# aouyang1/go-muse

Measured on AMD Instinct MI355X. Metric: series-pairs XCorr/sec at N=4096, 1M-series batch; achieved HBM GB/s, higher is better.
Workload: dtype f64

## Files before the change

### go-muse_amd/binding.py

```python
import ctypes
import os

import numpy as np

from . import build as _build

_i32 = ctypes.c_int32
_i64 = ctypes.c_int64
_f64 = ctypes.c_double
_vp = ctypes.c_void_p
_dp = ctypes.POINTER(ctypes.c_double)
_i32p = ctypes.POINTER(ctypes.c_int32)
_i64p = ctypes.POINTER(ctypes.c_int64)

MUSE_OK = 0
MUSE_ERR_INVALID = -1
MUSE_ERR_LENGTH = -2
MUSE_ERR_ZERO_STD = -3
MUSE_ERR_NO_DEVICE = -4
MUSE_ERR_HIP = -5
MUSE_ERR_UNSUPPORTED = -6
MUSE_ERR_NOMEM = -7
MUSE_ERR_EMPTY = -8
MUSE_LAG_WINDOW_MAX = 63
# ... 61 lines not shown
    "muse_merge_group_winners": (ctypes.c_int, [_recp, ctypes.POINTER(ctypes.c_uint8), _i32, _i32, _recp, ctypes.POINTER(ctypes.c_uint8)]),
    "muse_merge_records": (ctypes.c_int, [_recp, _i64, _i32, _i64p, _i32p, _dp, _i32p, _dp]),
    "muse_batch_score_many": (ctypes.c_int, [ctypes.POINTER(_vp), _i32]),
    "muse_batch_read_scores": (ctypes.c_int, [_vp, _i32p, _dp]),
    "muse_batch_last_run_info": (ctypes.c_int, [_vp, _i32p, _i64p]),
    "muse_batch_last_run_path": (ctypes.c_int, [_vp, _i32p]),
    "muse_batch_kernel_name": (ctypes.c_int, [_vp, ctypes.c_char_p, _i32]),
    "muse_test_set_screen_bound_scale": (ctypes.c_int, [_vp, _f64]),
    "muse_test_screen_bound": (ctypes.c_int, [_i32, _f64, _dp]),
    "muse_test_wave_argmax": (ctypes.c_int, [_vp, _dp, _dp, _dp]),
    "muse_test_rows_always_copy": (ctypes.c_int, [_vp, _i32]),
    "muse_test_pool_stats": (ctypes.c_int, [_vp, _i64p, _i64p, _i64p, _i64p]),
    "muse_test_xcorr_repeat": (ctypes.c_int, [_vp, _i32]),
    "muse_test_huge_batch_mb": (ctypes.c_int, [_vp, _i32]),
    "muse_test_clock_probe_start": (ctypes.c_int, [_vp, _f64, _f64]),
    "muse_test_clock_probe_stop": (ctypes.c_int, [_vp]),
    "muse_test_clock_probe_read": (ctypes.c_int, [_vp, _dp, _i32, _i32p]),
    "muse_batch_screen_estimates": (ctypes.c_int, [_vp, _i32, _dp, ctypes.POINTER(ctypes.c_uint32), _dp]),
    "muse_batch_score_many_windowed": (ctypes.c_int, [ctypes.POINTER(_vp), _i32, _i32]),
    "muse_batch_run_many_windowed": (ctypes.c_int, [ctypes.POINTER(_vp), _i32, _i32p, _i32, _i32, _i32, _f64, _i32, _i32,
                                                    _i64p, _i32p, _dp, _i32p, _dp]),
    "muse_test_window_many_plan": (ctypes.c_int, [_i32, _i32, _i32p, _i32p, _i32p, _i32p, _i32p, _i32p]),
    "muse_batch_run_many": (ctypes.c_int, [ctypes.POINTER(_vp), _i32, _i32p, _i32, _i32, _i32, _f64, _i32, _i32,
                                           _i64p, _i32p, _dp, _i32p, _dp]),
    "muse_batch_free": (ctypes.c_int, [_vp]),
    "muse_xcorr_with_x": (ctypes.c_int, [_vp, _dp, _dp, _i32, _i32, _dp, _i32p, _dp, _i32p]),
    "muse_xcorr": (ctypes.c_int, [_vp, _dp, _i32, _dp, _i32, _i32, _i32, _dp, _i32p, _dp, _i32p]),
    "muse_xcorr_groups": (ctypes.c_int, [_vp, _vp, _i32, _i32, _i32p, _dp, _i32p, _dp]),
    "muse_xcorr_batch": (ctypes.c_int, [_vp, _dp, _dp, _i64, _i32, _i32, _i32, _i32, _i32p, _dp, _i32p, _dp]),
    "muse_ctx_set_spectrum_cache": (ctypes.c_int, [_vp, _i32]),
    "muse_group_spectrum_cache": (ctypes.c_int, [_vp, _i64p, _i64p]),
    "muse_group_drop_spectrum_cache": (ctypes.c_int, [_vp]),
    "muse_test_spectrum_cache_limits": (ctypes.c_int, [_vp, _i64, _i64]),
    "muse_test_spectrum_cache_policy": (ctypes.c_int, [_i64, _i32, _i32, _i32, _i64, _i64, _i64, _i32p, _i64p, _i64p]),
    "muse_test_batch_redo_pairs": (ctypes.c_int, [_vp, _i64p, _i64, _i64p]),
    "muse_next_pow2": (_i64, [_f64]),
}


class MuseError(RuntimeError):
    def __init__(self, status, message):
        super().__init__("muse_hip status %d: %s" % (status, message))
        self.status = status
        self.message = message


_lib = None


def lib_path():
    return _build.LIB


def load():
    global _lib
    if _lib is None:
        path = lib_path()
        if not os.path.exists(path):
            raise MuseError(MUSE_ERR_NO_DEVICE,
                            "%s is not built; run `python -c 'import __graft_entry__ as g; g.build()'`" % path)
        L = ctypes.CDLL(path)
        for name, (res, args) in SIGNATURES.items():
            fn = getattr(L, name)
            fn.restype = res
            fn.argtypes = args
        _lib = L
# ... 28 lines not shown
```

### go-muse_amd/csrc/capi_batch.hip

```cpp
#include "capi_internal.h"
#include "xcorr_huge.h"

using namespace muse;


int ilog2(int64_t n)
{
    int l = 0;
    while (((int64_t)1 << l) < n)
        l++;
    return l;
}

int build_spectrum(muse_ctx *ctx, const double *ref_host, int N, int n, int normalize, double x_scale,
                          double xc_scale, double2 *X, double2 *xc, float2 *xcf, double *xs, int *zero_std)
{
    double *dref = nullptr;
    int *dstat = nullptr;
    double2 *dscr = nullptr;
    HIP_TRY(dmalloc(ctx, &dref, (size_t)N * sizeof(double)));
    hipError_t e = dmalloc(ctx, &dstat, sizeof(int));
    if (e == hipSuccess && n > GENERIC_LDS_MAX_N)
        e = dmalloc(ctx, &dscr, (size_t)n * sizeof(double2));
    if (e == hipSuccess)
// ... 467 lines not shown
        return fail(MUSE_ERR_INVALID, "NULL group");
    std::lock_guard<std::mutex> lock(g->ready_mu);
    if (rows_cached)
        *rows_cached = (g->zc_state == muse_group::ZC_VALID && g->zc_rewrites == g->rewrites) ? g->zc_rows : 0;
    if (bytes)
        *bytes = g->zc_bytes;
    return MUSE_OK;
}

extern "C" int muse_group_drop_spectrum_cache(muse_group *g)
{
    if (!g)
        return fail(MUSE_ERR_INVALID, "NULL group");
    std::lock_guard<std::mutex> lock(g->ready_mu);
    if (g->zc_segs.empty() && g->zc_state == muse_group::ZC_NONE)
        return MUSE_OK;
    int rc = use_device(g->ctx);
    if (rc)
        return rc;
    HIP_TRY(hipStreamSynchronize(g->ctx->stream));
    group_drop_spectrum_cache(g);
    return MUSE_OK;
}

extern "C" int muse_test_spectrum_cache_limits(muse_ctx *ctx, int64_t min_rows, int64_t budget_bytes)
{
    if (!ctx)
        return fail(MUSE_ERR_INVALID, "NULL context");
    ctx->zc_min_rows.store(min_rows < 0 ? ZC_MIN_ROWS : min_rows);
    ctx->zc_budget.store(budget_bytes < 0 ? -1 : budget_bytes);
    return MUSE_OK;
}

extern "C" int muse_test_spectrum_cache_policy(int64_t rows, int32_t N, int32_t f32, int32_t mode, int64_t min_rows,
                                               int64_t free_bytes, int64_t budget_bytes, int32_t *decision,
                                               int64_t *rows_cached, int64_t *bytes)
{
    if (!decision || !rows_cached || !bytes)
        return fail(MUSE_ERR_INVALID, "NULL output");
    *decision = spectrum_cache_policy(rows, N, f32 != 0, mode, min_rows < 0 ? ZC_MIN_ROWS : min_rows, free_bytes,
                                      budget_bytes < 0 ? -1 : budget_bytes, rows_cached, bytes);
    return MUSE_OK;
}

extern "C" int muse_test_batch_redo_pairs(muse_batch *b, int64_t *pairs, int64_t cap, int64_t *count)
{
    if (!b || !count || cap < 0 || (cap > 0 && !pairs))
        return fail(MUSE_ERR_INVALID, "bad redo-list arguments");
    *count = 0;
    int rc = use_device(b->ctx);
    if (rc)
        return rc;
    HIP_TRY(hipStreamSynchronize(b->stream()));
    if (!b->ovf_count || !b->ovf_list.p)
        return MUSE_OK;
    int listed = 0;
    HIP_TRY(hipMemcpy(&listed, b->ovf_count, sizeof(int), hipMemcpyDeviceToHost));
    *count = listed;
    const int64_t k = std::min<int64_t>(std::min<int64_t>(listed, cap), b->ovf_list.cap);
    if (k > 0)
        HIP_TRY(hipMemcpy(pairs, b->ovf_list.p, (size_t)k * sizeof(long long), hipMemcpyDeviceToHost));
    return MUSE_OK;
}

extern "C" int muse_batch_score(muse_batch *b)
{
// ... 42 lines not shown
        p.gsmall = kc.gsmall;
    if (variant == KERNEL_GENERIC && b->n <= GENERIC_LDS_MAX_N)
        p.gscratch = nullptr;
    LaunchTimer timer(ctx, false, st);
    LaunchTimer redo_timer(ctx, true, st);
    if (variant == KERNEL_R16_FOLD) {
        HIP_TRY(b->ovf_list.ensure(ctx, 2 * p.npairs, st));
        p.ovf_count = b->ovf_count;
        p.work_counter = b->ovf_count + 1;
        p.ovf_list = b->ovf_list.p;
        HIP_TRY(hipMemsetAsync(b->ovf_count, 0, 2 * sizeof(int), st));
        ZcPlan plan;
        std::unique_lock<std::mutex> zc_lock(b->g->ready_mu, std::defer_lock);
        if (allow_spectrum_cache && spectrum_cache_candidate(b, variant)) {
            zc_lock.lock();
            rc = plan_spectrum_cache(b, plan);
            if (rc)
                return rc;
            if (!plan.use)
                zc_lock.unlock();
        }
        HIP_TRY(timer.begin());
        if (plan.use) {
            bool launched = false;
            const auto next_launch = [&]() {
                const hipError_t e = launched ? hipMemsetAsync(b->ovf_count + 1, 0, sizeof(int), st) : hipSuccess;
                launched = true;
                return e;
            };
            for (const auto &sg : plan.readers) {
                FusedParams r = p;
                r.npairs = sg.pairs;
                HIP_TRY(next_launch());
                HIP_TRY(launch_cached(r, SpectrumCacheArgs{sg.zc(), sg.zstat(), sg.pair0, sg.pairs}, ctx->num_cus, st));
            }
            if (plan.tail_pair0 < p.npairs) {
                FusedParams w = p;
                w.npairs = p.npairs - plan.tail_pair0;
                HIP_TRY(next_launch());
                HIP_TRY(launch_cache_fill(w, SpectrumCacheArgs{plan.tail_zpairs ? plan.tail_seg.zc() : nullptr,
                                                               plan.tail_zpairs ? plan.tail_seg.zstat() : nullptr,
                                                               plan.tail_pair0, plan.tail_zpairs}, ctx->num_cus, st));
            }
            zc_lock.unlock();
        } else {
            HIP_TRY(launch_fused(p, variant, ctx->num_cus, st));
        }
        HIP_TRY(timer.end());
        FusedParams q = p;
        q.pair_list = b->ovf_list.p;
        q.pair_count = b->ovf_count;
        q.dense_total = ctx->variant == 0 ? p.npairs : 0;
        q.npairs = std::min<long long>(p.npairs, (long long)ctx->num_cus * 3);
        HIP_TRY(redo_timer.begin());
        HIP_TRY(launch_fused(q, KERNEL_R16_OCC3, ctx->num_cus, st));
        HIP_TRY(redo_timer.end());
        if (p.npairs >= 1024 && !(b->handoff_host && b->handoff_M == M && b->handoff_rewrites == b->g->rewrites)) {
            if (!b->handoff_host)
                HIP_TRY(hmalloc(ctx, &b->handoff_host, sizeof(int)));
            *b->handoff_host = 0;
            b->handoff_M = M;
            b->handoff_rewrites = b->g->rewrites;
            HIP_TRY(hipMemcpyAsync(b->handoff_host, b->ovf_count, sizeof(int), hipMemcpyDeviceToHost, st));
        }
    } else if (variant == KERNEL_LONG) {
        HIP_TRY(b->ovf_list.ensure(ctx, 2 * p.npairs, st));
        p.ovf_count = b->ovf_count;
// ... 28 lines not shown
    if (!lag || !mv)
        return fail(MUSE_ERR_INVALID, "NULL output");
    HIP_TRY(hipMemcpyAsync(lag, b->lag.p, (size_t)M * sizeof(int), hipMemcpyDeviceToHost, b->stream()));
    HIP_TRY(hipMemcpyAsync(mv, b->mv.p, (size_t)M * sizeof(double), hipMemcpyDeviceToHost, b->stream()));
    HIP_TRY(hipStreamSynchronize(b->stream()));
    return MUSE_OK;
}

extern "C" int muse_batch_kernel_name(muse_batch *b, char *name, int32_t cap)
{
    if (!b || !name || cap < 1)
        return fail(MUSE_ERR_INVALID, "NULL argument");
    char k[96] = "xcorr_fused_generic";
    const char *padded = b->N < b->n ? "true" : "false", *f32 = b->g->f32 ? "true" : "false";
    if (b->many_tiles > 0) {
        snprintf(k, sizeof(k), "xcorr_window_many_mfma<%d, %s>", b->many_tiles, window_wide(b->g->rows, b->g->stride) ? "true" : "false");
    } else if (b->windowed()) {
        const int L = std::min(b->lag_window, b->n / 2);
        snprintf(k, sizeof(k), "xcorr_window_mfma<%d, %s>", (2 * L + 1 + 15) / 16,
                 window_wide(b->g->rows, b->g->stride) ? "true" : "false");
    } else if (b->n > GENERIC_MAX_N) {
        snprintf(k, sizeof(k), "huge_rows<false>");
    } else {
        const KernelChoice kc = choose_kernel(b, (b->g->M + 1) / 2);
        switch (kc.error ? -1 : kc.variant) {
        case KERNEL_R16_FOLD: {
            bool cached = false;
            if (spectrum_cache_candidate(b, kc.variant)) {
                std::lock_guard<std::mutex> lock(b->g->ready_mu);
                int64_t rc_ = 0, by_ = 0;
                cached = b->g->zc_state == muse_group::ZC_VALID && b->g->zc_rewrites == b->g->rewrites && b->g->zc_rows > 0 &&
                         spectrum_cache_policy(b->g->M, b->N, false, b->ctx->zc_mode.load(), b->ctx->zc_min_rows.load(), 0, 0, &rc_, &by_) != ZC_POLICY_NONE;
            }
            if (cached)
                snprintf(k, sizeof(k), "xcorr_cached_n4096<%s>", padded);
            else
                snprintf(k, sizeof(k), "xcorr_fused_n4096_fold<false, %s, %s>", padded, f32);
            break;
        }
        case KERNEL_R16_OCC3: snprintf(k, sizeof(k), "xcorr_fused_n4096_occ4"); break;
        case KERNEL_SMALL: snprintf(k, sizeof(k), "xcorr_fused_small<%d, %s, false, %s>", b->logn, padded, f32); break;
        case KERNEL_LONG: snprintf(k, sizeof(k), "xcorr_fused_long<%d, %s, false>", b->logn, padded); break;
        case KERNEL_STOCKHAM: snprintf(k, sizeof(k), b->n >= 8192 ? "xcorr_fused_stk_4step" : "xcorr_fused_stockham"); break;
        case KERNEL_REAL_SPLIT: snprintf(k, sizeof(k), "xcorr_fused_real32k_split<%s>", padded); break;
        case KERNEL_REAL: snprintf(k, sizeof(k), "xcorr_fused_real%dk<%s>", b->n / 1024, padded); break;
        default: break;
        }
    }
    snprintf(name, (size_t)cap, "%s", k);
    return MUSE_OK;
}

extern "C" int muse_batch_free(muse_batch *b)
{
    if (!b)
        return MUSE_OK;
    muse_ctx *const c = b->ctx;
    (void)hipSetDevice(c->device);
    (void)hipStreamSynchronize(b->stream());
    if (b->sp && b->sp->refs.fetch_sub(1) == 1) {
        dfree(c, b->sp->X);
        dfree(c, b->sp->xc);
        dfree(c, b->sp->xcp);
        dfree(c, b->sp->xcw);
        dfree(c, b->sp->xcf);
        dfree(c, b->sp->xs);
        dfree(c, b->sp->c1);
        delete b->sp;
// ... 43 lines not shown
```

### go-muse_amd/csrc/capi_internal.h

```cpp
#pragma once
#include <hip/hip_runtime.h>

#include <algorithm>
#include <atomic>
#include <mutex>
#include <cmath>
#include <cstdarg>
#include <cstdio>
#include <cstdlib>
#include <cstring>
#include <ctime>
#include <limits>
#include <map>
#include <new>
#include <string>
#include <unordered_map>
#include <utility>
#include <vector>

#include "muse_hip.h"
#include "muse_hip_test.h"
#include "xcorr_kernels.h"

using namespace muse;
// ... 73 lines not shown
    std::vector<double *> stage_pool;
    std::mutex stage_mu;
    PoolBuf<double2> zscratch;
    PoolBuf<void *> many_tab;
    std::vector<void *> many_host;
    double screen_delta = 1e-4;
    int screening = 0;
    int64_t screen_min_rows = 0;
    double screen_e_scale = 1.0;
    int variant = 0;
    int xcorr_repeat = 1;
    unsigned long long *dbg_stamps = nullptr;
    hipStream_t probe_stream = nullptr;
    unsigned long long *probe_buf = nullptr;
    bool timing = false;
    std::vector<std::pair<hipEvent_t, hipEvent_t>> events, redo_events;
    double total_ms = 0.0, redo_ms = 0.0;
    int64_t launches = 0, redo_launches = 0;
    char pci[32] = {0};
    MemPool dev_pool, host_pool;
    HugeWork huge;
    int huge_batch_mb = 0;
    std::mutex huge_mu;
    std::mutex small_mu;
    std::vector<std::pair<unsigned char *, int>> small_free;
    unsigned long long small_token = 0;
    std::mutex timing_mu;
    std::atomic<bool> rows_always_copy{false};
    std::vector<void *> rows_slots;
    std::mutex rows_mu;
    std::atomic<int> zc_mode{1};
    std::atomic<int64_t> zc_min_rows{ZC_MIN_ROWS};
    std::atomic<int64_t> zc_budget{-1};
    std::atomic<int> win_rows_slices{0};
    std::atomic<bool> gather_nt{false};
    std::atomic<int> refs{1};
};

struct muse_group {
    std::atomic<int> refs{1};
    muse_ctx *ctx = nullptr;
    double *rows = nullptr;
    float *rows32 = nullptr;
    bool f32 = false;
    size_t elem() const { return f32 ? sizeof(float) : sizeof(double); }
    void *base() const { return f32 ? (void *)rows32 : (void *)rows; }
    int64_t cap = 0, M = 0, stride = 0;
    PoolBuf<double> hstats;
    int64_t hstats_rows = 0;
    uint64_t rewrites = 0;
    std::vector<void *> retired;
    int32_t N = 0;
    double *stage[2] = {nullptr, nullptr};
    hipEvent_t stage_done[2] = {nullptr, nullptr};
    int cur = 0;
    int64_t staged = 0;
    int64_t flushed = 0;
    int64_t stage_rows = 0;
    int small_appends = 0;
    int64_t win_rows = 0, win_committed = 0;
    std::mutex win_mu;
    hipEvent_t uploaded = nullptr;
    bool upload_pending = false;
    std::mutex ready_mu;
    HostBuf<long long> gidx_host;
    PoolBuf<long long> gidx_dev;
// ... 191 lines not shown
```

### go-muse_amd/csrc/foldk_device.h

```cpp
#pragma once
#include <hip/hip_runtime.h>
#include <stdint.h>

#include "fold_device.h"
#include "r16_device.h"

namespace muse {

namespace foldk {

using namespace occ4;
using namespace fold;

constexpr int XW = 544;

template <int PERM>
__device__ __forceinline__ constexpr int pr(int k)
{
    return PERM ? BR16(k) : k;
}

template <int MODE, int PERM, bool TAILBAR = false>
__device__ __forceinline__ void exchange_cross(double2 (&v)[16], double2 *xbuf, const int wave, const int t_, const int wcol = -1)
{
// ... 143 lines not shown
                 : [w0] "=&v"(w[0]), [w1] "=&v"(w[1]), [w2] "=&v"(w[2]), [w3] "=&v"(w[3]), [w4] "=&v"(w[4]),
                   [w5] "=&v"(w[5]), [w6] "=&v"(w[6]), [w7] "=&v"(w[7]), [w8] "=&v"(w[8]), [w9] "=&v"(w[9]),
                   [w10] "=&v"(w[10]), [w11] "=&v"(w[11]), [w12] "=&v"(w[12]), [w13] "=&v"(w[13]),
                   [w14] "=&v"(w[14]), [w15] "=&v"(w[15]), [sv] "=&s"(sv)
                 : [ra] "v"(raddr), [wa] "v"(waddr), [m] "s"(first), [d0] "v"(d[0]), [d1] "v"(d[1]), [d2] "v"(d[2]),
                   [d3] "v"(d[3]), [d4] "v"(d[4]), [d5] "v"(d[5]), [d6] "v"(d[6]), [d7] "v"(d[7])
                 : "memory", "scc");
#pragma unroll
    for (int e = 0; e < 16; e++)
        v[e] = make_double2(w[e].x, w[e].y);
}

struct G2Fetch {
    const double2 *p;
    int j;
    __device__ __forceinline__ double2 operator()(int s) const { return p[16 * s + j]; }
};
struct G3Fetch {
    const double2 *p;
    int t;
    __device__ __forceinline__ double2 operator()(int s) const
    {
        return ldg2(scalar_ptr_at(p, ((s + 1) & ~1) * 256), t - 256 * (s & 1));
    }
};

struct G3Derived {
    double2 g[8];
    __device__ __forceinline__ static double2 sq(const double2 w) { return make_double2(fma_(w.x, w.x, -(w.y * w.y)), (w.x + w.x) * w.y); }
    __device__ __forceinline__ static double2 mulc(const double2 w, const double c, const double s)
    {
        return make_double2(fma_(w.y, s, w.x * c), fma_(-w.x, s, w.y * c));
    }
    __device__ __forceinline__ G3Derived(const double2 *tab, int t)
    {
        constexpr double H = 0.70710678118654752440;
        const double2 w8 = G3Fetch{tab, t}(2), w16 = G3Fetch{tab, t}(4);
        g[2] = w8;
        g[4] = w16;
        g[1] = sq(w8);
        g[0] = sq(g[1]);
        g[3] = make_double2(H * (w8.x + w8.y), H * (w8.y - w8.x));
        g[5] = mulc(w16, C16_1, S16_1);
        g[6] = make_double2(H * (w16.x + w16.y), H * (w16.y - w16.x));
        g[7] = mulc(w16, S16_1, C16_1);
    }
    __device__ __forceinline__ double2 operator()(int s) const { return g[s]; }
};

template <typename F>
__device__ __forceinline__ void gdft16_nr_l2(double2 (&v)[16], F fetch)
{
    double2 ga[4], gb[4];
#pragma unroll
    for (int s = 0; s < 4; s++)
        ga[s] = fetch(s);
    gdft16_nr_s12(v, ga[0], ga[1]);
    fence();
#pragma unroll
    for (int s = 0; s < 4; s++)
        gb[s] = fetch(4 + s);
    fence();
    gdft16_nr_s3(v, ga[2], ga[3]);
    fence();
    fence();
    gdft16_nr_s4(v, gb[0], gb[1], gb[2], gb[3]);
}

constexpr int REC = 36;

// ... 192 lines not shown
```

### go-muse_amd/csrc/xcorr_kernels.h

```cpp
#pragma once
#include <hip/hip_runtime.h>
#include <stdint.h>

#include "muse_hip.h"

namespace muse {

enum { KERNEL_GENERIC = 0, KERNEL_R16_OCC3 = 6, KERNEL_STOCKHAM = 10, KERNEL_R16_FOLD = 11, KERNEL_SMALL = 12, KERNEL_LONG = 13, KERNEL_REAL = 14, KERNEL_REAL_SPLIT = 15 };

struct FusedParams {
    const double *rows;
    const float *rows32;
    long long M;
    long long stride;
    long long npairs;
    int N;
    int n;
    int logn;
    int normalize_y;
    const double2 *xc;
    const double2 *tw1;
    const double2 *tw2;
    const double2 *xcp;
    const double2 *g2;
// ... 38 lines not shown
    const long long *pair_list;
    const int *pair_count;
    long long dense_total;
    long long gscratch_slices;
    const double *xrows;
    long long xstride;
    int Nx;
    double invN, invNm1;
};
inline FusedParams with_reciprocals(FusedParams p)
{
    p.invN = 1.0 / (double)p.N;
    p.invNm1 = 1.0 / (double)(p.N - 1);
    return p;
}

hipError_t launch_fused(const FusedParams &p, int variant, int num_cus, hipStream_t stream);
hipError_t launch_fused_occ4(const FusedParams &p, int num_cus, hipStream_t stream);
hipError_t launch_screen_pass(const FusedParams &p, int num_cus, hipStream_t stream);
hipError_t launch_screen_pass_many(const FusedParams &p, int num_cus, hipStream_t stream);
hipError_t launch_screen_pass_stk(const FusedParams &p, int num_cus, hipStream_t stream);
enum : unsigned { SCR_IN = 1u, SCR_OUT = 2u, SCR_POS = 4u, SCR_NEG = 8u, SCR_REFINE = 16u, SCR_NAN = 32u };
hipError_t launch_fused_fold(const FusedParams &p, int num_cus, hipStream_t stream);
hipError_t launch_fused_multi(const FusedParams &p, int num_cus, hipStream_t stream);
constexpr int ZC_STAT = 16;
constexpr long long ZC_PAIR_BYTES = 4096 * 16 + ZC_STAT * 8;
struct SpectrumCacheArgs {
    double2 *zc;
    double *zstat;
    long long pair0;
    long long zpairs;
};
hipError_t launch_cache_fill(const FusedParams &p, const SpectrumCacheArgs &c, int num_cus, hipStream_t stream);
hipError_t launch_cached(const FusedParams &p, const SpectrumCacheArgs &c, int num_cus, hipStream_t stream);
hipError_t launch_fused_small(const FusedParams &p, int num_cus, hipStream_t stream);
hipError_t launch_fused_stockham(const FusedParams &p, int num_cus, hipStream_t stream);
hipError_t launch_fused_long(const FusedParams &p, int num_cus, hipStream_t stream);
hipError_t launch_real_split_tables(const double2 *xc, double2 *out, hipStream_t stream);
hipError_t launch_real8k_tables(const double2 *xc, double2 *out, hipStream_t stream);
hipError_t launch_two_sided_real(const FusedParams &p, int num_cus, hipStream_t stream);
hipError_t launch_fused_real_split(const FusedParams &p, int num_cus, hipStream_t stream);
hipError_t launch_fused_real(const FusedParams &p, int num_cus, hipStream_t stream);
hipError_t launch_two_sided(const FusedParams &p, int num_cus, hipStream_t stream);
hipError_t launch_two_sided_small(const FusedParams &p, int num_cus, hipStream_t stream);
hipError_t launch_lane_order_rows(const double2 *in, double2 *out, int R1, hipStream_t stream);
hipError_t launch_lane_order(const double2 *in, double2 *out, hipStream_t stream);
hipError_t launch_indicator_corr(const double *xs, int n, int pad, double *c1, hipStream_t stream);
hipError_t launch_ref_spectrum(const double *ref_dev, int N, int n, int logn, int normalize, double x_scale,
                               double xc_scale, const double2 *twm, double2 *X, double2 *xc, float2 *xcf, double *xs,
                               double2 *gscratch, int *status, hipStream_t stream);
constexpr int SMALL_MAX_N = 16384;
constexpr int GENERIC_LDS_MAX_N = 8192;
constexpr int GENERIC_MAX_N = 65536;
constexpr int GENERIC_GLOBAL_WGS_PER_CU = 2;
constexpr int STOCKHAM_GLOBAL_WGS_PER_CU = 2;
constexpr int LONG_WGS_PER_CU = 4;
constexpr int GSCRATCH_SLICES_PER_CU = 4;
static_assert(LONG_WGS_PER_CU <= GSCRATCH_SLICES_PER_CU && GENERIC_GLOBAL_WGS_PER_CU <= GSCRATCH_SLICES_PER_CU &&
                  2 * STOCKHAM_GLOBAL_WGS_PER_CU <= GSCRATCH_SLICES_PER_CU,
              "the scratch buffer is sized for GSCRATCH_SLICES_PER_CU slices per CU");
constexpr int WIN_KC = 1024;
constexpr int WIN_E_TAIL = 128;
static_assert(2 * MUSE_LAG_WINDOW_MAX + 2 <= WIN_E_TAIL, "the staged image covers every lag of the widest window");
struct WindowParams {
    const double *rows;
    long long M, stride;
    int N;
// ... 143 lines not shown
```

### go-muse_amd/csrc/xcorr_r16_cached.hip

```cpp
#include <hip/hip_runtime.h>
#include <stdint.h>
#include <algorithm>

#include "foldk_device.h"

namespace muse {

namespace foldk {

#if defined(__HIP_DEVICE_COMPILE__)
typedef d2v __attribute__((address_space(1))) *zc_out_ptr;
typedef double __attribute__((address_space(1))) *zstat_out_ptr;
typedef const double __attribute__((address_space(4))) *zstat_in_ptr;
#endif

__device__ __forceinline__ void finalize_prev(const double *prec, const int wave, const int lane, const double invN,
                                              const double invNm1, const FusedParams &p)
{
    if (lane == 0 && wave < 2 && prec[34] >= 0.0 && (wave == 0 || prec[35] != 0.0)) {
        const long long row = (long long)prec[34] + wave;
        if (finalize(prec, wave, invN, invNm1, p.mv + row, p.lag + row)) {
            const int slot = atomicAdd(p.ovf_count, 1);
            p.ovf_list[slot] = row >> 1;
        }
    }
}

}

template <bool PADDED>
__global__ __launch_bounds__(OCC_THREADS, 4) void xcorr_cache_fill_n4096(const FusedParams p, const SpectrumCacheArgs c)
{
    using namespace occ4;
    using namespace fold;
    using namespace foldk;
    __shared__ double2 xbuf[OCC_XBUF];
    __shared__ double2 g2s[128];
    __shared__ double red[2 * REC];
    __shared__ int next_s[2];
    const int t = threadIdx.x;
    const int lane = t & 63;
    const int wave = __builtin_amdgcn_readfirstlane(t >> 6);
    double2 *const xw = xbuf + XW * wave;
    const int pad = PADDED ? 4096 - p.N : 0;
    const double invN = PADDED ? p.invN : 1.0 / 4096.0, invNm1 = PADDED ? p.invNm1 : 1.0 / 4095.0;

// ... 108 lines not shown
                    cq[k] = c1l(8 * h + k);
                fence();
#pragma unroll
                for (int k = 0; k < 8; k++) {
                    const int r = BR16(8 * h + k);
                    v[r] = make_double2(fma(-mA, cq[k], v[r].x), fma(-mB, cq[k], v[r].y));
                }
            }
        }
        wave_argmax_store(v, wave, lane, rec + 6 * wave);
        fence();
        request_rows(nxt);
        fence();
        if (wave == 0 && lane == 0) {
            rec[32] = s1a;
            rec[33] = s1b;
        }
        parity ^= 1;
    }
    lds_barrier();
    {
        const double *const prec = red + REC * (parity ^ 1);
        if (t < 2 && prec[34] >= 0.0 && (t == 0 || prec[35] != 0.0)) {
            const long long row = (long long)prec[34] + t;
            if (finalize(prec, t, invN, invNm1, p.mv + row, p.lag + row)) {
                const int slot = atomicAdd(p.ovf_count, 1);
                p.ovf_list[slot] = row >> 1;
            }
        }
    }
}

template <bool PADDED>
__global__ __launch_bounds__(OCC_THREADS, 4) void xcorr_cached_n4096(const FusedParams p, const SpectrumCacheArgs c)
{
    using namespace occ4;
    using namespace fold;
    using namespace foldk;
    __shared__ double2 xbuf[OCC_XBUF];
    __shared__ double2 g2s[128];
    __shared__ double red[2 * REC];
    __shared__ int next_s[2];
    const int t = threadIdx.x;
    const int lane = t & 63;
    const int wave = __builtin_amdgcn_readfirstlane(t >> 6);
    double2 *const xw = xbuf + XW * wave;
    const double invN = PADDED ? p.invN : 1.0 / 4096.0, invNm1 = PADDED ? p.invNm1 : 1.0 / 4095.0;

    if (t < 128)
        g2s[t] = p.g2[t];
    if (t < 2)
        red[REC * (t) + 34] = -1.0;
    __syncthreads();
    const auto tl = [&]() __attribute__((always_inline)) {
        int x = t;
        if (PADDED)
            asm volatile("" : "+v"(x));
        return x;
    };

    int parity = 0;
    const long long first = c.pair0, total = c.pair0 + p.npairs;
    d2v zn[16];
    const auto request_z = [&](long long pr) __attribute__((always_inline)) {
#pragma unroll
        for (int i = 0; i < 16; i++)
            zn[i] = __builtin_nontemporal_load((gptr<d2v>)scalar_ptr_at(c.zc, (pr - first) * 4096 + 256 * ((i + 1) & ~1)) + (t - 256 * (i & 1)));
    };
    request_z(first + blockIdx.x < total ? first + (long long)blockIdx.x : first);

    long long nextpair = 0;
    for (long long pair = first + blockIdx.x; pair < total; pair = nextpair) {
        const long long rA = 2 * pair;
        const bool hasB = rA + 1 < p.M;
        double *const rec = red + REC * parity;
        const double *const prec = red + REC * (parity ^ 1);
        if (t == 0)
            next_s[parity] = (int)gridDim.x + atomicAdd(p.work_counter, 1);
        double st[10];
#if defined(__HIP_DEVICE_COMPILE__)
        {
            const zstat_in_ptr sp = (zstat_in_ptr)(unsigned long long)(c.zstat + (pair - first) * ZC_STAT);
#pragma unroll
            for (int k = 0; k < 10; k++)
                st[k] = sp[k];
        }
#endif
        double2 v[16];
#pragma unroll
        for (int i = 0; i < 16; i++)
            v[i] = make_double2(zn[i].x, zn[i].y);
        xc_stage1(v, [&](int j) __attribute__((always_inline)) {
            return ldg2(scalar_ptr_at(p.xcp, 256 * ((j + 1) & ~1)), t - 256 * (j & 1));
        });
        dft16_rn_s234(v);
        exchange_local<0>(v, xw, tl());
        gdft16_nr(v, G2Fetch{g2s, t & 15});
// ... 18 lines not shown
#pragma unroll
            for (int h = 0; h < 2; h++) {
                double cq[8];
#pragma unroll
                for (int k = 0; k < 8; k++)
                    cq[k] = c1l(8 * h + k);
                fence();
#pragma unroll
                for (int k = 0; k < 8; k++) {
                    const int r = BR16(8 * h + k);
                    v[r] = make_double2(fma(-mA, cq[k], v[r].x), fma(-mB, cq[k], v[r].y));
                }
            }
        }
        wave_argmax_store(v, wave, lane, rec + 6 * wave);
        fence();
        request_z(nxt);
        fence();
        parity ^= 1;
    }
    lds_barrier();
    {
        const double *const prec = red + REC * (parity ^ 1);
        if (t < 2 && prec[34] >= 0.0 && (t == 0 || prec[35] != 0.0)) {
            const long long row = (long long)prec[34] + t;
            if (finalize(prec, t, invN, invNm1, p.mv + row, p.lag + row)) {
                const int slot = atomicAdd(p.ovf_count, 1);
                p.ovf_list[slot] = row >> 1;
            }
        }
    }
}

static bool cache_launch_ok(const FusedParams &p, const SpectrumCacheArgs &c)
{
    return p.rows && !p.rows32 && p.n == 4096 && p.N > 2048 && p.N <= 4096 && p.npairs > 0 && c.pair0 >= 0 &&
           2 * (c.pair0 + p.npairs) <= p.M + 1 && p.work_counter && p.ovf_count && p.ovf_list && p.g2 && p.g3a && p.g3b && p.xcp &&
           (p.N == 4096 || p.c1);
}

hipError_t launch_cache_fill(const FusedParams &p_in, const SpectrumCacheArgs &c, int num_cus, hipStream_t stream)
{
    const FusedParams p = with_reciprocals(p_in);
    if (!cache_launch_ok(p, c) || c.zpairs < 0 || c.zpairs > p.npairs || (c.zpairs > 0 && (!c.zc || !c.zstat)) ||
        2 * (c.pair0 + c.zpairs) > p.M)
        return hipErrorInvalidValue;
    const dim3 g((unsigned)std::min<long long>(p.npairs, (long long)num_cus * 4)), b(OCC_THREADS);
    if (p.N < 4096)
        hipLaunchKernelGGL((xcorr_cache_fill_n4096<true>), g, b, 0, stream, p, c);
    else
        hipLaunchKernelGGL((xcorr_cache_fill_n4096<false>), g, b, 0, stream, p, c);
    return hipGetLastError();
}

hipError_t launch_cached(const FusedParams &p_in, const SpectrumCacheArgs &c, int num_cus, hipStream_t stream)
{
    const FusedParams p = with_reciprocals(p_in);
    if (!cache_launch_ok(p, c) || !c.zc || !c.zstat || c.zpairs < p.npairs || 2 * (c.pair0 + p.npairs) > p.M)
        return hipErrorInvalidValue;
    const dim3 g((unsigned)std::min<long long>(p.npairs, (long long)num_cus * 4)), b(OCC_THREADS);
    if (p.N < 4096)
        hipLaunchKernelGGL((xcorr_cached_n4096<true>), g, b, 0, stream, p, c);
    else
        hipLaunchKernelGGL((xcorr_cached_n4096<false>), g, b, 0, stream, p, c);
    return hipGetLastError();
}

}
```

### go-muse_amd/muse.py

```python
import ctypes
import math
import sys
import threading
import uuid
import weakref

import numpy as np

from . import binding as B
from .binding import MuseError

DefaultLabel = "uid"

SignFilter_POS = 1
SignFilter_NEG = -1
SignFilter_ANY = 0


class Engine:

    def __init__(self, device=0):
        self._h = ctypes.c_void_p()
        B.check(B.load().muse_ctx_create(int(device), ctypes.byref(self._h)))
        self.device = int(device)
# ... 12 lines not shown
            B.load().muse_ctx_destroy(self._h)
            self._h = ctypes.c_void_p()

    def __del__(self):
        try:
            if not sys.is_finalizing():
                self.close()
        except Exception:
            pass

    def synchronize(self):
        B.check(B.load().muse_ctx_synchronize(self._h))

    def device_info(self):
        name = ctypes.create_string_buffer(128)
        cus, hbm = ctypes.c_int32(0), ctypes.c_int64(0)
        B.check(B.load().muse_ctx_device_info(self._h, name, 128, ctypes.byref(cus), ctypes.byref(hbm)))
        return name.value.decode(), int(cus.value), int(hbm.value)

    def set_kernel(self, variant):
        B.check(B.load().muse_ctx_set_kernel(self._h, int(variant)))

    def set_screening(self, enable, min_rows=None):
        B.check(B.load().muse_ctx_set_screening(self._h, (int(min_rows) if min_rows and min_rows > 1 else 1) if enable else 0))

    def set_screen_bound_scale(self, scale):
        B.check(B.load().muse_test_set_screen_bound_scale(self._h, float(scale)))

    def set_spectrum_cache(self, on):
        B.check(B.load().muse_ctx_set_spectrum_cache(self._h, 1 if on else 0))

    def spectrum_cache_limits(self, min_rows=-1, budget_bytes=-1):
        B.check(B.load().muse_test_spectrum_cache_limits(self._h, int(min_rows), int(budget_bytes)))

    def trim(self):
        B.check(B.load().muse_ctx_trim(self._h))

    def pool_stats(self):
        v = [ctypes.c_int64(0) for _ in range(4)]
        B.check(B.load().muse_test_pool_stats(self._h, *[ctypes.byref(x) for x in v]))
        return tuple(int(x.value) for x in v)

    def xcorr_repeat(self, repeat):
        B.check(B.load().muse_test_xcorr_repeat(self._h, int(repeat)))

    def huge_batch_mb(self, megabytes):
        B.check(B.load().muse_test_huge_batch_mb(self._h, int(megabytes)))

    def rows_always_copy(self, on):
        B.check(B.load().muse_test_rows_always_copy(self._h, 1 if on else 0))

    def window_rows_slices(self, S):
        B.check(B.load().muse_test_window_rows_slices(self._h, int(S)))

    def wave_argmax(self, cc_a, cc_b):
        a = np.ascontiguousarray(cc_a, dtype=np.float64)
        b = np.ascontiguousarray(cc_b, dtype=np.float64)
        if a.shape != (4096,) or b.shape != (4096,):
            raise ValueError("wave_argmax: two vectors of 4096 values")
        out = np.zeros(24)
        B.check(B.load().muse_test_wave_argmax(self._h, B.dptr(a), B.dptr(b), B.dptr(out)))
        return out.reshape(4, 2, 3)

    def clock_probe_start(self, window_ms=1.0, total_ms=1000.0):
        B.check(B.load().muse_test_clock_probe_start(self._h, float(window_ms), float(total_ms)))

# ... 1181 lines not shown
```

Baseline: 138.5 million.

## Add deep-pipelined cached spectrum reader with lower occupancy as default

Adds a deep variant of the cached-spectrum xcorr kernel and makes it the default for both padded and full lengths. The deep variant prefetches the next pair's spectrum and stats while the current one is computed, keeps g3 twiddles in registers for the full-length case, and runs at 2 blocks per CU instead of 4. The aim is to hide HBM latency through in-thread prefetch instead of relying on occupancy. The cost is higher register pressure and fewer resident waves, so latency hiding now depends on the software pipeline. A test hook selects the lean or deep form.

```diff
diff --git a/go-muse_amd/binding.py b/go-muse_amd/binding.py
--- a/go-muse_amd/binding.py
+++ b/go-muse_amd/binding.py
@@ -117,6 +117,7 @@
     "muse_group_spectrum_cache": (ctypes.c_int, [_vp, _i64p, _i64p]),
     "muse_group_drop_spectrum_cache": (ctypes.c_int, [_vp]),
     "muse_test_spectrum_cache_limits": (ctypes.c_int, [_vp, _i64, _i64]),
+    "muse_test_cached_reader": (ctypes.c_int, [_vp, _i32]),
     "muse_test_spectrum_cache_policy": (ctypes.c_int, [_i64, _i32, _i32, _i32, _i64, _i64, _i64, _i32p, _i64p, _i64p]),
     "muse_test_batch_redo_pairs": (ctypes.c_int, [_vp, _i64p, _i64, _i64p]),
     "muse_next_pow2": (_i64, [_f64]),
diff --git a/go-muse_amd/csrc/capi_batch.hip b/go-muse_amd/csrc/capi_batch.hip
--- a/go-muse_amd/csrc/capi_batch.hip
+++ b/go-muse_amd/csrc/capi_batch.hip
@@ -523,6 +523,14 @@
     return MUSE_OK;
 }
 
+extern "C" int muse_test_cached_reader(muse_ctx *ctx, int32_t form)
+{
+    if (!ctx || form < CACHED_READER_DEFAULT || form > CACHED_READER_DEEP)
+        return fail(MUSE_ERR_INVALID, "cached reader form is 0 (default), 1 (lean) or 2 (deep)");
+    ctx->zc_reader.store(form);
+    return MUSE_OK;
+}
+
 extern "C" int muse_test_spectrum_cache_policy(int64_t rows, int32_t N, int32_t f32, int32_t mode, int64_t min_rows,
                                                int64_t free_bytes, int64_t budget_bytes, int32_t *decision,
                                                int64_t *rows_cached, int64_t *bytes)
@@ -631,7 +639,7 @@
                 FusedParams r = p;
                 r.npairs = sg.pairs;
                 HIP_TRY(next_launch());
-                HIP_TRY(launch_cached(r, SpectrumCacheArgs{sg.zc(), sg.zstat(), sg.pair0, sg.pairs}, ctx->num_cus, st));
+                HIP_TRY(launch_cached(r, SpectrumCacheArgs{sg.zc(), sg.zstat(), sg.pair0, sg.pairs}, ctx->zc_reader.load(), ctx->num_cus, st));
             }
             if (plan.tail_pair0 < p.npairs) {
                 FusedParams w = p;
@@ -726,8 +734,12 @@
                 cached = b->g->zc_state == muse_group::ZC_VALID && b->g->zc_rewrites == b->g->rewrites && b->g->zc_rows > 0 &&
                          spectrum_cache_policy(b->g->M, b->N, false, b->ctx->zc_mode.load(), b->ctx->zc_min_rows.load(), 0, 0, &rc_, &by_) != ZC_POLICY_NONE;
             }
-            if (cached)
-                snprintf(k, sizeof(k), "xcorr_cached_n4096<%s>", padded);
+            if (cached) {
+                const int form = b->ctx->zc_reader.load();
+                const bool is_padded = b->N < b->n, deep = cached_reader_is_deep(form, is_padded);
+                snprintf(k, sizeof(k), "xcorr_cached%s_n4096<%s>",
+                         deep == cached_reader_is_deep(CACHED_READER_DEFAULT, is_padded) ? "" : (deep ? "_deep" : "_lean"), padded);
+            }
             else
                 snprintf(k, sizeof(k), "xcorr_fused_n4096_fold<false, %s, %s>", padded, f32);
             break;
diff --git a/go-muse_amd/csrc/capi_internal.h b/go-muse_amd/csrc/capi_internal.h
--- a/go-muse_amd/csrc/capi_internal.h
+++ b/go-muse_amd/csrc/capi_internal.h
@@ -129,6 +129,7 @@
     std::atomic<int> zc_mode{1};
     std::atomic<int64_t> zc_min_rows{ZC_MIN_ROWS};
     std::atomic<int64_t> zc_budget{-1};
+    std::atomic<int> zc_reader{0};
     std::atomic<int> win_rows_slices{0};
     std::atomic<bool> gather_nt{false};
     std::atomic<int> refs{1};
diff --git a/go-muse_amd/csrc/foldk_device.h b/go-muse_amd/csrc/foldk_device.h
--- a/go-muse_amd/csrc/foldk_device.h
+++ b/go-muse_amd/csrc/foldk_device.h
@@ -199,10 +199,10 @@
     {
         return make_double2(fma_(w.y, s, w.x * c), fma_(-w.x, s, w.y * c));
     }
-    __device__ __forceinline__ G3Derived(const double2 *tab, int t)
+    __device__ __forceinline__ G3Derived(const double2 *tab, int t) : G3Derived(G3Fetch{tab, t}(2), G3Fetch{tab, t}(4)) {}
+    __device__ __forceinline__ G3Derived(const double2 w8, const double2 w16)
     {
         constexpr double H = 0.70710678118654752440;
-        const double2 w8 = G3Fetch{tab, t}(2), w16 = G3Fetch{tab, t}(4);
         g[2] = w8;
         g[4] = w16;
         g[1] = sq(w8);
diff --git a/go-muse_amd/csrc/xcorr_kernels.h b/go-muse_amd/csrc/xcorr_kernels.h
--- a/go-muse_amd/csrc/xcorr_kernels.h
+++ b/go-muse_amd/csrc/xcorr_kernels.h
@@ -94,7 +94,14 @@
     long long zpairs;
 };
 hipError_t launch_cache_fill(const FusedParams &p, const SpectrumCacheArgs &c, int num_cus, hipStream_t stream);
-hipError_t launch_cached(const FusedParams &p, const SpectrumCacheArgs &c, int num_cus, hipStream_t stream);
+enum { CACHED_READER_DEFAULT = 0, CACHED_READER_LEAN = 1, CACHED_READER_DEEP = 2 };
+constexpr bool CACHED_DEEP_DEFAULT_FULL = true;
+constexpr bool CACHED_DEEP_DEFAULT_PADDED = true;
+constexpr bool cached_reader_is_deep(int form, bool padded)
+{
+    return form == CACHED_READER_DEEP || (form == CACHED_READER_DEFAULT && (padded ? CACHED_DEEP_DEFAULT_PADDED : CACHED_DEEP_DEFAULT_FULL));
+}
+hipError_t launch_cached(const FusedParams &p, const SpectrumCacheArgs &c, int form, int num_cus, hipStream_t stream);
 hipError_t launch_fused_small(const FusedParams &p, int num_cus, hipStream_t stream);
 hipError_t launch_fused_stockham(const FusedParams &p, int num_cus, hipStream_t stream);
 hipError_t launch_fused_long(const FusedParams &p, int num_cus, hipStream_t stream);
diff --git a/go-muse_amd/csrc/xcorr_r16_cached.hip b/go-muse_amd/csrc/xcorr_r16_cached.hip
--- a/go-muse_amd/csrc/xcorr_r16_cached.hip
+++ b/go-muse_amd/csrc/xcorr_r16_cached.hip
@@ -12,6 +12,7 @@
 typedef d2v __attribute__((address_space(1))) *zc_out_ptr;
 typedef double __attribute__((address_space(1))) *zstat_out_ptr;
 typedef const double __attribute__((address_space(4))) *zstat_in_ptr;
+typedef int __attribute__((address_space(1))) *counter_ptr;
 #endif
 
 __device__ __forceinline__ void finalize_prev(const double *prec, const int wave, const int lane, const double invN,
@@ -186,7 +187,7 @@
 }
 
 template <bool PADDED>
-__global__ __launch_bounds__(OCC_THREADS, 4) void xcorr_cached_n4096(const FusedParams p, const SpectrumCacheArgs c)
+__device__ __forceinline__ void cached_lean_body(const FusedParams &p, const SpectrumCacheArgs &c)
 {
     using namespace occ4;
     using namespace fold;
@@ -217,6 +218,9 @@
     const long long first = c.pair0, total = c.pair0 + p.npairs;
     d2v zn[16];
     const auto request_z = [&](long long pr) __attribute__((always_inline)) {
+#ifdef MUSE_ABLATE_CACHED_L2HOT
+        pr = first;
+#endif
 #pragma unroll
         for (int i = 0; i < 16; i++)
             zn[i] = __builtin_nontemporal_load((gptr<d2v>)scalar_ptr_at(c.zc, (pr - first) * 4096 + 256 * ((i + 1) & ~1)) + (t - 256 * (i & 1)));
@@ -301,6 +305,163 @@
     }
 }
 
+template <bool PADDED>
+__device__ __forceinline__ void cached_deep_body(const FusedParams &p, const SpectrumCacheArgs &c)
+{
+    using namespace occ4;
+    using namespace fold;
+    using namespace foldk;
+    __shared__ double2 xbuf[OCC_XBUF_FULL];
+    __shared__ double2 g2s[128];
+    __shared__ double red[2 * REC];
+    __shared__ int next_s[2];
+    const int t = threadIdx.x;
+    const int lane = t & 63;
+    const int wave = __builtin_amdgcn_readfirstlane(t >> 6);
+    double2 *const xw = xbuf + 1088 * wave;
+    const double invN = PADDED ? p.invN : 1.0 / 4096.0, invNm1 = PADDED ? p.invNm1 : 1.0 / 4095.0;
+
+    if (t < 128)
+        g2s[t] = p.g2[t];
+    if (t < 2)
+        red[REC * (t) + 34] = -1.0;
+    __syncthreads();
+
+    int parity = 0;
+    const long long first = c.pair0, total = c.pair0 + p.npairs;
+    d2v zn[16];
+    double stv;
+    const auto request_z = [&](long long pr) __attribute__((always_inline)) {
+#ifdef MUSE_ABLATE_CACHED_L2HOT
+        pr = first;
+#endif
+#pragma unroll
+        for (int i = 0; i < 16; i++)
+            zn[i] = __builtin_nontemporal_load((gptr<d2v>)scalar_ptr_at(c.zc, (pr - first) * 4096 + 256 * ((i + 1) & ~1)) + (t - 256 * (i & 1)));
+    };
+    const auto request_stat = [&](long long pr) __attribute__((always_inline)) {
+#ifdef MUSE_ABLATE_CACHED_L2HOT
+        pr = first;
+#endif
+        stv = scalar_ptr_at(c.zstat, (pr - first) * ZC_STAT)[lane & 15];
+    };
+    long long pair = first + blockIdx.x, nextpair = first + (long long)gridDim.x + blockIdx.x;
+    request_z(pair < total ? pair : first);
+    request_stat(pair < total ? pair : first);
+    double2 xf[16];
+#pragma unroll
+    for (int j = 0; j < 16; j++)
+        xf[j] = ldg2(scalar_ptr_at(p.xcp, 256 * ((j + 1) & ~1)), t - 256 * (j & 1));
+    constexpr bool G3_RESIDENT = !PADDED;
+    double2 w8 = make_double2(0.0, 0.0), w16 = w8;
+    if (G3_RESIDENT) {
+        w8 = G3Fetch{p.g3b, t}(2);
+        w16 = G3Fetch{p.g3b, t}(4);
+    }
+
+#pragma clang loop unroll(disable)
+    for (; pair < total;) {
+        const long long rA = 2 * pair;
+        const bool hasB = rA + 1 < p.M;
+        double *const rec = red + REC * parity;
+        const double *const prec = red + REC * (parity ^ 1);
+        int claim = 0;
+#if defined(__HIP_DEVICE_COMPILE__)
+        if (t == 0) {
+            counter_ptr wc = (counter_ptr)(unsigned long long)p.work_counter;
+            asm volatile("" : "+v"(wc));
+            claim = __hip_atomic_fetch_add(wc, 1, __ATOMIC_RELAXED, __HIP_MEMORY_SCOPE_AGENT);
+        }
+#endif
+        double2 v[16];
+#pragma unroll
+        for (int i = 0; i < 16; i++)
+            v[i] = make_double2(zn[i].x, zn[i].y);
+        xc_stage1_pre(v, xf);
+        fence();
+        request_z(nextpair < total ? nextpair : first);
+        fence();
+        dft16_rn_s234(v);
+        exchange_local_full<0>(v, xw, t);
+        gdft16_nr(v, G2Fetch{g2s, t & 15});
+        if (t == 0)
+            next_s[parity] = 2 * (int)gridDim.x + claim;
+        exchange_cross_full<1, 1>(v, xbuf, t);
+        finalize_prev(prec, wave, lane, invN, invNm1, p);
+        if (t < 10)
+            rec[24 + t] = stv;
+        if (t == 0) {
+            rec[34] = (double)rA;
+            rec[35] = hasB ? 1.0 : 0.0;
+        }
+        const long long claimed = first + __builtin_amdgcn_readfirstlane(next_s[parity]);
+        if (G3_RESIDENT) {
+            double2 g8 = w8, g16 = w16;
+            asm volatile("" : "+v"(g8.x), "+v"(g8.y), "+v"(g16.x), "+v"(g16.y));
+            gdft16_nr_l2(v, G3Derived(g8, g16));
+        } else {
+            gdft16_nr_l2(v, G3Derived(p.g3b, t));
+        }
+        if (PADDED) {
+            const auto c1l = [&](int k) __attribute__((always_inline)) {
+                return scalar_ptr_at(p.c1, 256 * ((k + 1) & ~1))[t - 256 * (k & 1)];
+            };
+            const double mA = readlane_f64(stv, 8) * invN, mB = readlane_f64(stv, 9) * invN;
+#pragma unroll
+            for (int h = 0; h < 4; h++) {
+                double cq[4];
+#pragma unroll
+                for (int k = 0; k < 4; k++)
+                    cq[k] = c1l(4 * h + k);
+                fence();
+#pragma unroll
+                for (int k = 0; k < 4; k++) {
+                    const int r = BR16(4 * h + k);
+                    v[r] = make_double2(fma(-mA, cq[k], v[r].x), fma(-mB, cq[k], v[r].y));
+                }
+            }
+        }
+        fence();
+        request_stat(nextpair < total ? nextpair : first);
+        fence();
+        wave_argmax_store(v, wave, lane, rec + 6 * wave);
+        pair = nextpair;
+        nextpair = claimed;
+        parity ^= 1;
+    }
+    lds_barrier();
+    {
+        const double *const prec = red + REC * (parity ^ 1);
+        if (t < 2 && prec[34] >= 0.0 && (t == 0 || prec[35] != 0.0)) {
+            const long long row = (long long)prec[34] + t;
+            if (finalize(prec, t, invN, invNm1, p.mv + row, p.lag + row)) {
+                const int slot = atomicAdd(p.ovf_count, 1);
+                p.ovf_list[slot] = row >> 1;
+            }
+        }
+    }
+}
+
+constexpr bool cached_deep_default(bool padded) { return padded ? CACHED_DEEP_DEFAULT_PADDED : CACHED_DEEP_DEFAULT_FULL; }
+template <bool PADDED>
+__global__ __launch_bounds__(OCC_THREADS, cached_deep_default(PADDED) ? 2 : 4) void xcorr_cached_n4096(const FusedParams p, const SpectrumCacheArgs c)
+{
+    if constexpr (cached_deep_default(PADDED))
+        cached_deep_body<PADDED>(p, c);
+    else
+        cached_lean_body<PADDED>(p, c);
+}
+template <bool PADDED>
+__global__ __launch_bounds__(OCC_THREADS, 4) void xcorr_cached_lean_n4096(const FusedParams p, const SpectrumCacheArgs c)
+{
+    cached_lean_body<PADDED>(p, c);
+}
+template <bool PADDED>
+__global__ __launch_bounds__(OCC_THREADS, 2) void xcorr_cached_deep_n4096(const FusedParams p, const SpectrumCacheArgs c)
+{
+    cached_deep_body<PADDED>(p, c);
+}
+
 static bool cache_launch_ok(const FusedParams &p, const SpectrumCacheArgs &c)
 {
     return p.rows && !p.rows32 && p.n == 4096 && p.N > 2048 && p.N <= 4096 && p.npairs > 0 && c.pair0 >= 0 &&
@@ -322,16 +483,29 @@
     return hipGetLastError();
 }
 
-hipError_t launch_cached(const FusedParams &p_in, const SpectrumCacheArgs &c, int num_cus, hipStream_t stream)
+template <bool PADDED>
+static void launch_cached_form(bool deep, dim3 g, dim3 b, hipStream_t stream, const FusedParams &p, const SpectrumCacheArgs &c)
+{
+    if (deep == cached_deep_default(PADDED))
+        hipLaunchKernelGGL((xcorr_cached_n4096<PADDED>), g, b, 0, stream, p, c);
+    else if constexpr (cached_deep_default(PADDED))
+        hipLaunchKernelGGL((xcorr_cached_lean_n4096<PADDED>), g, b, 0, stream, p, c);
+    else
+        hipLaunchKernelGGL((xcorr_cached_deep_n4096<PADDED>), g, b, 0, stream, p, c);
+}
+
+hipError_t launch_cached(const FusedParams &p_in, const SpectrumCacheArgs &c, int form, int num_cus, hipStream_t stream)
 {
     const FusedParams p = with_reciprocals(p_in);
-    if (!cache_launch_ok(p, c) || !c.zc || !c.zstat || c.zpairs < p.npairs || 2 * (c.pair0 + p.npairs) > p.M)
+    if (!cache_launch_ok(p, c) || !c.zc || !c.zstat || c.zpairs < p.npairs || 2 * (c.pair0 + p.npairs) > p.M ||
+        form < CACHED_READER_DEFAULT || form > CACHED_READER_DEEP)
         return hipErrorInvalidValue;
-    const dim3 g((unsigned)std::min<long long>(p.npairs, (long long)num_cus * 4)), b(OCC_THREADS);
+    const bool deep = cached_reader_is_deep(form, p.N < 4096);
+    const dim3 g((unsigned)std::min<long long>(p.npairs, (long long)num_cus * (deep ? 2 : 4))), b(OCC_THREADS);
     if (p.N < 4096)
-        hipLaunchKernelGGL((xcorr_cached_n4096<true>), g, b, 0, stream, p, c);
+        launch_cached_form<true>(deep, g, b, stream, p, c);
     else
-        hipLaunchKernelGGL((xcorr_cached_n4096<false>), g, b, 0, stream, p, c);
+        launch_cached_form<false>(deep, g, b, stream, p, c);
     return hipGetLastError();
 }
 
diff --git a/go-muse_amd/muse.py b/go-muse_amd/muse.py
--- a/go-muse_amd/muse.py
+++ b/go-muse_amd/muse.py
@@ -68,6 +68,9 @@
 
     def spectrum_cache_limits(self, min_rows=-1, budget_bytes=-1):
         B.check(B.load().muse_test_spectrum_cache_limits(self._h, int(min_rows), int(budget_bytes)))
+
+    def cached_reader(self, form=0):
+        B.check(B.load().muse_test_cached_reader(self._h, int(form)))
 
     def trim(self):
         B.check(B.load().muse_ctx_trim(self._h))
```

Result: faster. 145.1 million, median of 6 (+4.8%).
